# fabsig/GPBoost

Hardware: AMD Instinct MI355X
Metric: neg-log-lik evals/sec, n=1000000 Vecchia(m=30) fp64 (higher is better)
Workload: dtype f64

## Files before the change

### gpboost_amd/csrc/dev_common.h

```cpp
#pragma once
#include <hip/hip_runtime.h>
#include <stdint.h>
#include <type_traits>
#include <utility>

namespace gpb {

template <int B, int E, class F>
__device__ __forceinline__ void static_for(F&& f) {
  if constexpr (B < E) {
    f(std::integral_constant<int, B>{});
    static_for<B + 1, E>(f);
  }
}
template <int B, int E, class F>
__device__ __forceinline__ void static_for_down(F&& f) {
  if constexpr (B < E) {
    f(std::integral_constant<int, E - 1>{});
    static_for_down<B, E - 1>(f);
  }
}

template <int LANE>
__device__ __forceinline__ double row_bcast(double x) {
  static_assert(LANE >= 0 && LANE < 16, "row_newbcast lane");
  double r;
  asm volatile("s_nop 1\n\tv_mov_b64_dpp %0, %1 row_newbcast:%2 row_mask:0xf bank_mask:0xf"
               : "=v"(r)
               : "v"(x), "n"(LANE));
  return r;
}
template <int LANE>
__device__ __forceinline__ void row_fnma(double& acc, double b, double own) {
  static_assert(LANE >= 0 && LANE < 16, "row_newbcast lane");
#ifdef GPB_DPP_PAD_EVERY_FMAC
  asm volatile("s_nop 1\n\tv_fmac_f64_dpp %0, -%1, %2 row_newbcast:%3 row_mask:0xf bank_mask:0xf"
               : "+v"(acc)
               : "v"(b), "v"(own), "n"(LANE));
#else
  asm volatile("v_fmac_f64_dpp %0, -%1, %2 row_newbcast:%3 row_mask:0xf bank_mask:0xf"
               : "+v"(acc)
               : "v"(b), "v"(own), "n"(LANE));
#endif
}
__device__ __forceinline__ void dpp_fence(double& a) { asm volatile("s_nop 1" : "+v"(a)); }
__device__ __forceinline__ void dpp_fence(double& a, double& b) { asm volatile("s_nop 1" : "+v"(a), "+v"(b)); }
__device__ __forceinline__ void dpp_fence(double& a, double& b, double& c) { asm volatile("s_nop 1" : "+v"(a), "+v"(b), "+v"(c)); }
__device__ __forceinline__ void dpp_fence(double& a, double& b, double& c, double& d) { asm volatile("s_nop 1" : "+v"(a), "+v"(b), "+v"(c), "+v"(d)); }
template <int CTRL>
__device__ __forceinline__ double dpp_move_f64(double v) {
  const long long b = __builtin_bit_cast(long long, v);
  int lo = (int)(b & 0xffffffffll), hi = (int)(b >> 32);
  lo = __builtin_amdgcn_update_dpp(0, lo, CTRL, 0xF, 0xF, true);
  hi = __builtin_amdgcn_update_dpp(0, hi, CTRL, 0xF, 0xF, true);
  return __builtin_bit_cast(double, ((long long)hi << 32) | (long long)(unsigned int)lo);
}
__device__ __forceinline__ double row_sum16(double v) {
  v += dpp_move_f64<0xB1>(v);
  v += dpp_move_f64<0x4E>(v);
  v += dpp_move_f64<0x141>(v);
  v += dpp_move_f64<0x140>(v);
  return v;
}
__host__ __device__ constexpr unsigned long long row_lanes_le(int j) {
  return j < 0 ? 0ull : (j >= 15 ? ~0ull : ((1ull << (j + 1)) - 1ull) * 0x0001000100010001ull);
}
__host__ __device__ constexpr unsigned long long row_lane_eq(int j) { return (1ull << j) * 0x0001000100010001ull; }
template <unsigned long long MASK>
__device__ __forceinline__ int sel_lanes(int a, int b, int tok) {
  int r;
  asm("s_mov_b32 vcc_lo, %3\n\ts_mov_b32 vcc_hi, %4\n\tv_cndmask_b32_e32 %0, %1, %2, vcc ; %5"
      : "=v"(r) : "v"(b), "v"(a), "n"((int)(unsigned)(MASK & 0xffffffffull)), "n"((int)(unsigned)(MASK >> 32)), "s"(tok) : "vcc");
  return r;
}
template <unsigned long long MASK, int A, int B>
__device__ __forceinline__ int sel_lanes_const(int tok) {
  static_assert(A >= 0 && A <= 64 && B >= 0 && B <= 64, "inline constants only");
  int r;
  asm("s_mov_b32 vcc_lo, %3\n\ts_mov_b32 vcc_hi, %4\n\tv_cndmask_b32_e64 %0, %1, %2, vcc ; %5"
      : "=v"(r) : "n"(B), "n"(A), "n"((int)(unsigned)(MASK & 0xffffffffull)), "n"((int)(unsigned)(MASK >> 32)), "s"(tok) : "vcc");
  return r;
}
template <unsigned long long MASK>
__device__ __forceinline__ void set_lanes(double& dst, double v) {
  asm volatile("s_mov_b32 exec_lo, %2\n\ts_mov_b32 exec_hi, %3\n\tv_mov_b64 %0, %1\n\ts_mov_b64 exec, -1"
               : "+v"(dst) : "v"(v), "n"((int)(unsigned)(MASK & 0xffffffffull)), "n"((int)(unsigned)(MASK >> 32)));
}
template <int LANE>
__device__ __forceinline__ double row_bcast_builtin(double x) {
  const long long v = __builtin_bit_cast(long long, x);
  int lo = (int)(v & 0xffffffffll), hi = (int)(v >> 32);
  lo = __builtin_amdgcn_update_dpp(0, lo, 0x150 + LANE, 0xf, 0xf, false);
  hi = __builtin_amdgcn_update_dpp(0, hi, 0x150 + LANE, 0xf, 0xf, false);
  const long long r = ((long long)hi << 32) | (unsigned long long)(unsigned int)lo;
  return __builtin_bit_cast(double, r);
}
#ifdef GPB_DPP_VIA_BUILTIN
#define GPB_ROW_BCAST(L, x) ::gpb::row_bcast_builtin<L>(x)
#define GPB_ROW_FNMA(L, acc, b, own) (acc) = __builtin_fma(-::gpb::row_bcast_builtin<L>(b), (own), (acc))
#else
#define GPB_ROW_BCAST(L, x) ::gpb::row_bcast<L>(x)
#define GPB_ROW_FNMA(L, acc, b, own) ::gpb::row_fnma<L>((acc), (b), (own))
#endif


__device__ __forceinline__ double fast_rcp(double x) {
  const double y0 = __builtin_amdgcn_rcp(x);
  const double e = __builtin_fma(-x, y0, 1.0);
  return __builtin_fma(y0, e, y0);
}

#ifndef GPB_EXP_TAB_SIZE
#define GPB_EXP_TAB_SIZE 256
#endif
static_assert(GPB_EXP_TAB_SIZE == 256, "exp_of_scaled is written for a 256-entry table");

enum CovType : int { kMatern05 = 0, kMatern15 = 1, kMatern25 = 2 };

constexpr double kLn2OverT = 0.0027076061740622863;
constexpr double kCoordScale = 184.6649652337873;

struct KernEval { double ev, rp; };
__device__ __forceinline__ KernEval exp_of_scaled(double d2q, const double* __restrict__ tabv) {
  const double h = __builtin_amdgcn_rsq(d2q);
  const double g = d2q * h;
  const double e = __builtin_fma(-h, g, 3.0);
  const double rp = g * e;
  const double kf = __builtin_rint(-rp);
  const double rr = -rp - kf;
  const int k = (int)kf;
  double p = __builtin_fma(rr, 2.239395190875157e-12, 3.3083026805413713e-09);
  p = __builtin_fma(p, rr, 3.6655655969101062e-06);
  p = __builtin_fma(p, rr, kLn2OverT);
  p = __builtin_fma(p, rr, 1.0);
  KernEval o;
  o.ev = __builtin_ldexp(tabv[k & (GPB_EXP_TAB_SIZE - 1)] * p, k >> 8);
  o.rp = rp;
  return o;
}
template <int COV>
__device__ __forceinline__ double matern_cov_s(double d2s, const double* __restrict__ tabv) {
  const KernEval k = exp_of_scaled(d2s, tabv);
  if constexpr (COV == kMatern05) return k.ev;
  else if constexpr (COV == kMatern15) return k.ev * __builtin_fma(k.rp, kLn2OverT, 1.0);
  else { const double r = k.rp * kLn2OverT; return k.ev * __builtin_fma(r, __builtin_fma(r, 1.0 / 3.0, 1.0), 1.0); }
}
template <int COV>
__device__ __forceinline__ double matern_cov_dlog_s(double d2s, const double* __restrict__ tabv, double& dk) {
  const KernEval k = exp_of_scaled(d2s, tabv);
  const double r = k.rp * kLn2OverT;
  if constexpr (COV == kMatern05) { dk = -r * k.ev; return k.ev; }
  else if constexpr (COV == kMatern15) { dk = -(r * r) * k.ev; return k.ev * (1.0 + r); }
  else { dk = -(1.0 / 3.0) * (r * r) * (1.0 + r) * k.ev; return k.ev * __builtin_fma(r, __builtin_fma(r, 1.0 / 3.0, 1.0), 1.0); }
}
template <int COV>
__device__ __forceinline__ double matern_dlog_range_s(double d2s, const double* __restrict__ tabv) {
  const KernEval k = exp_of_scaled(d2s, tabv);
  const double r = k.rp * kLn2OverT;
  if constexpr (COV == kMatern05) return -r * k.ev;
  else if constexpr (COV == kMatern15) return -(r * r) * k.ev;
  else return -(1.0 / 3.0) * (r * r) * __builtin_fma(1.0, r, 1.0) * k.ev;
}

}
```

### gpboost_amd/csrc/vecchia_kernels.hip

```cpp
#include <algorithm>
#include "dev_common.h"
#include "vecchia_kernels.h"

namespace gpb {

namespace {

constexpr double kDummyCoord = 1e30;

__host__ __device__ constexpr int lane_of_row(int r) { return ((r / 16) & 1) ? 15 - (r % 16) : (r % 16); }

template <int MT>
struct Layout {
  static_assert(MT >= 1 && MT <= 62, "1 <= MT <= 62");
  static_assert(MT % 16 != 15, "row MT and row MT+1 must share a register slot");
  static constexpr int R = MT + 2;
  static constexpr int NS = (R + 15) / 16;
  static constexpr int PS = MT / 16, PL = lane_of_row(MT);
  static constexpr int YS = (MT + 1) / 16, YL = lane_of_row(MT + 1);
  static constexpr int NCOL = MT + 1;
  static constexpr int PTS_BYTES32 = (NS * 16) * 32 + 16;
  static constexpr int PTS_STRIDE24 = NS * 16 + 2;
  __host__ __device__ static constexpr int cmax(int s) { return (16 * s + 15 < MT) ? 16 * s + 15 : MT; }
};

template <bool D3> struct RecT;
template <> struct RecT<true> { double x, y, z, w; __device__ __forceinline__ double zz() const { return z; } };
template <> struct RecT<false> { double x, y, w; __device__ __forceinline__ double zz() const { return 0.0; } };

template <bool D3>
__device__ __forceinline__ double sq_dist_s(double px, double py, double pz, double qx, double qy, double qz) {
  const double dx = px - qx, dy = py - qy;
  double d2 = __builtin_fma(dx, dx, 1e-300);
  d2 = __builtin_fma(dy, dy, d2);
  if constexpr (D3) {
    const double dz = pz - qz;
    d2 = __builtin_fma(dz, dz, d2);
  }
  return d2;
}

template <int MT>
__host__ __device__ constexpr int num_lower_steps() {
  using L = Layout<MT>;
  int n = 8 * L::NS * (L::NS - 1) + 15 * (L::NS / 2);
  if (L::NS & 1) { const int s = L::NS - 1; const int chi = (16 * s + 14 < MT - 1) ? 16 * s + 14 : MT - 1; n += chi - 16 * s + 1; }
  return n;
}
template <int MT, class FR, class FP, class FS>
__device__ __forceinline__ void for_each_lower_step(FR&& rect, FP&& pair, FS&& solo) {
  using L = Layout<MT>;
  constexpr int RECT_TOTAL = 8 * L::NS * (L::NS - 1);
  static_for<1, L::NS>([&](auto s_) {
    constexpr int s = decltype(s_)::value;
    static_for<0, 16 * s>([&](auto c_) { rect(s_, c_, std::integral_constant<int, 8 * s * (s - 1) + decltype(c_)::value>{}); });
  });
  static_for<0, L::NS>([&](auto s_) {
    constexpr int s = decltype(s_)::value;
    if constexpr ((s & 1) == 1) {
      static_for<0, 15>([&](auto j_) {
        constexpr int j = decltype(j_)::value;
        constexpr int cA = 16 * s + j, cB = 16 * (s - 1) + 14 - j;
        using E = std::integral_constant<int, RECT_TOTAL + 15 * (s / 2) + j>;
        if constexpr (cA <= MT - 1) pair(s_, std::integral_constant<int, cA>{}, std::integral_constant<int, s - 1>{},
                                         std::integral_constant<int, cB>{}, std::integral_constant<int, 14 - j>{}, E{});
        else solo(std::integral_constant<int, s - 1>{}, std::integral_constant<int, cB>{}, E{});
      });
    } else if constexpr (s == L::NS - 1) {
      constexpr int chi = (16 * s + 14 < MT - 1) ? 16 * s + 14 : MT - 1;
      static_for<16 * s, chi + 1>([&](auto c_) { solo(s_, c_, std::integral_constant<int, RECT_TOTAL + 15 * (L::NS / 2) + decltype(c_)::value - 16 * s>{}); });
    }
  });
}

}

constexpr unsigned long long kGranuleEmpty = ~0ull;
template <int NP>
__device__ __forceinline__ void vecchia_finish(const VecchiaKernelArgs& args, int G, double (*s_fin)[4]);

template <int MT, int MODE>
constexpr bool kRuntimeWeightedInstance() { return MODE == MODE_GRAD && MT > 30 && MT <= 40; }

template <int MT, int COV, bool D3, int MODE, bool WT>
__global__ __launch_bounds__(256, (MT > 30 && MT <= 40 && MODE != MODE_NLL) ? 2 : 1) void vecchia_point_kernel(VecchiaKernelArgs args) {
  using L = Layout<MT>;
  constexpr int NS = L::NS;
  constexpr bool kNeedSolve = (MODE != MODE_NLL);
#ifdef GPB_NLL_RIGHT_LOOKING
  constexpr bool kLeftLooking = false;
#else
  constexpr bool kLeftLooking = MT > 30 && (!kNeedSolve || NS == 3);
#endif
  constexpr bool kLeftSolve = kLeftLooking && kNeedSolve;
  constexpr int NP = (MODE == MODE_GRAD) ? GPB_NUM_PARTIALS : 3;

  using Rec = RecT<D3>;
  constexpr bool kStoreDK = (MODE == MODE_GRAD) && (MT <= 30);
  constexpr int NSTEP = num_lower_steps<MT>();
  constexpr bool kLastDkInReg = kStoreDK && D3;
  constexpr int NSTORE = kStoreDK ? (kLastDkInReg ? NSTEP - 1 : NSTEP) : 1;
  constexpr int PBYTES = D3 ? L::PTS_BYTES32 : L::PTS_STRIDE24 * (int)sizeof(Rec);
  __shared__ double s_tab[GPB_EXP_TAB_SIZE];
  __shared__ __attribute__((aligned(16))) char s_pts_raw[16 * PBYTES];
  __shared__ double s_red[GPB_NUM_PARTIALS][16];
  __shared__ double s_f0[kLeftSolve ? 16 : 1][kLeftSolve ? 256 : 1];
  constexpr bool kDgInLds = WT && (MODE == MODE_NLL) && kLeftLooking;
  __shared__ double s_dg[kDgInLds ? 16 : 1][kDgInLds ? NS * 16 : 1];
  __shared__ double s_dk[NSTORE][kStoreDK ? 256 : 1];
  static_assert(PBYTES % 16 == 0 && PBYTES >= 16 * (NS * 16), "record block: 16-byte aligned, room for the (A, b) pairs");
  __shared__ double2 s_ab[(MODE == MODE_GRAD && !kStoreDK) ? 16 : 1][(MODE == MODE_GRAD && !kStoreDK) ? NS * 16 : 1];
  double dk_last = 0.0;

  __shared__ double s_tot[GPB_NUM_PARTIALS];
  __shared__ double s_fin[GPB_NUM_PARTIALS][4];

  const int G = (int)gridDim.x - 1;
  if ((int)blockIdx.x == G) { vecchia_finish<NP>(args, G, s_fin); return; }
  const int tid0 = threadIdx.x;
  static_assert(GPB_EXP_TAB_SIZE == 256, "one table entry per thread");
  s_tab[tid0] = args.exp_tab[tid0] * args.var;
  if (tid0 < NP) s_tot[tid0] = 0.0;
  __shared__ double s_pm[16];
  __shared__ int s_pe[16];
  if (tid0 < 16) { s_pm[tid0] = 0.5; s_pe[tid0] = 1; }

  const int m = args.m;
  auto fetch_idx = [&](int grp_, int tid_, int (&out)[NS]) {
    const int g_ = tid_ >> 4, l_ = tid_ & 15;
    const long long ir = (long long)args.i_begin + (long long)grp_ * 16 + g_;
    const int ii = ir < (long long)args.i_end ? (int)ir : args.i_end - 1;
#pragma unroll
    for (int s = 0; s < NS; ++s) {
      const int r = 16 * s + ((s & 1) ? 15 - l_ : l_);
      int idx = -1;
      if (r < m) idx = args.nn[(size_t)ii * m + r];
      else if (r == MT) idx = ii;
      out[s] = idx;
    }
  };
  int nidx[NS];
  fetch_idx(blockIdx.x, tid0, nidx);
  for (int grp = blockIdx.x; grp < args.ngroups; grp += G) {
  int tid = tid0;
  asm volatile("; per-trip thread index" : "+v"(tid));
  const int g = tid >> 4;
  const int l = tid & 15;
  const long long i_raw = (long long)args.i_begin + (long long)grp * 16 + g;
  const bool active = i_raw < (long long)args.i_end;
  const int i = active ? (int)i_raw : args.i_end - 1;
  int cidx[NS];
#pragma unroll
  for (int s = 0; s < NS; ++s) cidx[s] = nidx[s];
  if (grp + G < args.ngroups) fetch_idx(grp + G, tid, nidx);
  const double sc = args.a * kCoordScale;

  const double4 ctr = args.pts[i];
  Rec own[NS];
  constexpr bool kRuntimeW = WT && kRuntimeWeightedInstance<MT, MODE>();
  const bool weighted = kRuntimeW ? (args.nug != nullptr) : WT;
  constexpr int kOwnDg = (kDgInLds || !WT) ? 1 : NS;
  double own_dg[kOwnDg];
#pragma unroll
  for (int s = 0; s < kOwnDg; ++s) own_dg[s] = 0.0;
  auto own_dg_of = [&](int s) -> double { if constexpr (kOwnDg == NS) return own_dg[s]; else { (void)s; return own_dg[0]; } };
#pragma unroll
  for (int s = 0; s < NS; ++s) {
    const int r = 16 * s + ((s & 1) ? 15 - l : l);
    const int idx = cidx[s];
    if (WT && weighted) {
      const double dgv = args.var + (idx >= 0 ? args.nug[idx] : 1.0);
      if constexpr (kDgInLds) s_dg[g][r] = dgv; else own_dg[s] = dgv;
    }
    Rec p;
    if (idx >= 0) {
      const double4 q = args.pts[idx];
      p.x = (q.x - ctr.x) * sc; p.y = (q.y - ctr.y) * sc; p.w = q.w;
      if constexpr (D3) p.z = (q.z - ctr.z) * sc;
    } else {
      p.x = kDummyCoord * (double)(r + 1); p.y = 0.0; p.w = 0.0;
      if constexpr (D3) p.z = 0.0;
    }
    own[s] = p;
    reinterpret_cast<Rec*>(s_pts_raw + g * PBYTES)[r] = p;
  }
  __syncthreads();
  const double* tabv = s_tab;
  const Rec* gp = reinterpret_cast<const Rec*>(s_pts_raw + g * PBYTES);
  int row_off[NS];
#pragma unroll
  for (int s = 0; s < NS; ++s) row_off[s] = (16 * s + ((s & 1) ? 15 - l : l)) * (int)sizeof(Rec);

  double M[NS][L::NCOL];
  auto eval_entry = [&](const Rec& o, const Rec& q, auto e_) -> double {
    const double d2 = sq_dist_s<D3>(o.x, o.y, o.zz(), q.x, q.y, q.zz());
    if constexpr (kStoreDK) {
      double dk;
      const double v = matern_cov_dlog_s<COV>(d2, tabv, dk);
      if constexpr (kLastDkInReg && decltype(e_)::value == NSTEP - 1) dk_last = dk;
      else s_dk[decltype(e_)::value][tid] = dk;
      return v;
    } else {
      return matern_cov_s<COV>(d2, tabv);
    }
  };
  if constexpr (kLeftLooking) {
    auto eval_plain = [&](const Rec& o, const Rec& q) -> double {
      return matern_cov_s<COV>(sq_dist_s<D3>(o.x, o.y, o.zz(), q.x, q.y, q.zz()), tabv);
    };
    static_for<0, MT + 1>([&](auto c_) {
      constexpr int c = decltype(c_)::value;
      constexpr int sc_ = c / 16, lc = lane_of_row(c);
      if constexpr (c < MT) {
        static_for<sc_ + 1, NS>([&](auto s_) { constexpr int s = decltype(s_)::value; M[s][c] = eval_plain(own[s], gp[c]); });
        if constexpr ((c % 16) != 15 && (sc_ & 1) == 0) {
          constexpr int j = 14 - (c - 16 * sc_);
          constexpr int sA = sc_ + 1, cA = 16 * sA + j;
          if constexpr (sA < NS && cA <= MT - 1) {
            constexpr unsigned long long MA = row_lanes_le(14 - j);
            const int ro = sel_lanes<MA>(row_off[sA], row_off[sc_], grp);
            const int co = sel_lanes_const<MA, cA, c>(grp) * (int)sizeof(Rec);
            const double v = eval_plain(*reinterpret_cast<const Rec*>(reinterpret_cast<const char*>(gp) + ro),
                                        *reinterpret_cast<const Rec*>(reinterpret_cast<const char*>(gp) + co));
            M[sA][cA] = v;
            M[sc_][c] = v;
          } else {
            M[sc_][c] = eval_plain(own[sc_], gp[c]);
          }
        }
      }
      {
        double dg;
        if constexpr (kDgInLds) dg = weighted ? s_dg[g][c] : ((c == MT) ? args.diag_i : args.diag_nn);
        else dg = weighted ? own_dg_of(sc_) : ((c == MT) ? args.diag_i : args.diag_nn);
        if constexpr (c == 16 * sc_ + 15 || c == MT) M[sc_][c] = dg;
        else set_lanes<row_lane_eq(lc)>(M[sc_][c], dg);
        set_lanes<row_lane_eq(L::YL)>(M[L::YS][c], gp[c].w);
      }
      static_for<0, c>([&](auto k_) {
        constexpr int k = decltype(k_)::value;
        static_for<sc_, NS>([&](auto s_) {
          constexpr int s = decltype(s_)::value;
          GPB_ROW_FNMA(lc, M[s][c], M[sc_][k], M[s][k]);
        });
      });
      if constexpr (c < MT) {
        const double piv = GPB_ROW_BCAST(lc, M[sc_][c]);
        const double y0 = __builtin_amdgcn_rsq(piv);
        const double e = __builtin_fma(-0.5 * piv * y0, y0, 0.5);
        const double rs = __builtin_fma(y0, e, y0);
        static_for<sc_, NS>([&](auto s_) { constexpr int s = decltype(s_)::value; M[s][c] *= rs; });
        if constexpr (kLeftSolve) set_lanes<row_lane_eq(lc)>(M[sc_][c], rs);
        static_assert(NS <= 4, "dpp_fence overloads cover four slots");
        if constexpr (NS - sc_ == 1) dpp_fence(M[sc_][c]);
        else if constexpr (NS - sc_ == 2) dpp_fence(M[sc_][c], M[sc_ + 1][c]);
        else if constexpr (NS - sc_ == 3) dpp_fence(M[sc_][c], M[sc_ + 1][c], M[sc_ + 2][c]);
        else dpp_fence(M[sc_][c], M[sc_ + 1][c], M[sc_ + 2][c], M[sc_ + 3][c]);
        if constexpr (kLeftSolve && c == 15) static_for<0, 16>([&](auto q_) { s_f0[decltype(q_)::value][tid] = M[0][decltype(q_)::value]; });
      }
    });
  } else {
  for_each_lower_step<MT>(
      [&](auto s_, auto c_, auto e_) {
        constexpr int s = decltype(s_)::value, c = decltype(c_)::value;
        M[s][c] = eval_entry(own[s], gp[c], e_);
      },
      [&](auto sA_, auto cA_, auto sB_, auto cB_, auto J_, auto e_) {
        constexpr int sA = decltype(sA_)::value, cA = decltype(cA_)::value, sB = decltype(sB_)::value,
                      cB = decltype(cB_)::value, J = decltype(J_)::value;
        constexpr unsigned long long MA = row_lanes_le(J);
        const int ro = sel_lanes<MA>(row_off[sA], row_off[sB], grp);
        const int co = sel_lanes_const<MA, cA, cB>(grp) * (int)sizeof(Rec);
        const Rec o = *reinterpret_cast<const Rec*>(reinterpret_cast<const char*>(gp) + ro);
        const Rec q = *reinterpret_cast<const Rec*>(reinterpret_cast<const char*>(gp) + co);
        const double v = eval_entry(o, q, e_);
        M[sA][cA] = v;
        M[sB][cB] = v;
      },
      [&](auto s_, auto c_, auto e_) {
        constexpr int s = decltype(s_)::value, c = decltype(c_)::value;
        M[s][c] = eval_entry(own[s], gp[c], e_);
      });
  static_for<0, NS>([&](auto s_) {
    constexpr int s = decltype(s_)::value;
    static_for<16 * s, L::cmax(s) + 1>([&](auto c_) {
      constexpr int c = decltype(c_)::value;
      double dg;
      if constexpr (kDgInLds) dg = weighted ? s_dg[g][c] : ((c == MT) ? args.diag_i : args.diag_nn);
      else dg = weighted ? own_dg_of(s) : ((c == MT) ? args.diag_i : args.diag_nn);
      if constexpr (c == 16 * s + 15 || c == MT) M[s][c] = dg;
      else set_lanes<row_lane_eq(lane_of_row(c))>(M[s][c], dg);
    });
  });
  if (l == L::YL) {
    static_for<0, MT + 1>([&](auto c_) { M[L::YS][decltype(c_)::value] = gp[decltype(c_)::value].w; });
  }

  static_for<0, MT>([&](auto k_) {
    constexpr int k = decltype(k_)::value;
    constexpr int sk = k / 16, lk = lane_of_row(k);
    if constexpr (k == 0) static_for<0, NS>([&](auto s_) { dpp_fence(M[decltype(s_)::value][0]); });
    const double piv = GPB_ROW_BCAST(lk, M[sk][k]);
    const double inv = fast_rcp(piv);
    double T[NS];
    static_for<sk, NS>([&](auto s_) { T[decltype(s_)::value] = M[decltype(s_)::value][k] * inv; });
    static_for<k + 1, MT + 1>([&](auto c_) {
      constexpr int c = decltype(c_)::value;
      constexpr int sc_ = c / 16, lc = lane_of_row(c);
      static_for<sc_, NS>([&](auto s_) {
        constexpr int s = decltype(s_)::value;
        GPB_ROW_FNMA(lc, M[s][c], M[sc_][k], T[s]);
      });
    });
    if constexpr (kNeedSolve) static_for<sk, NS>([&](auto s_) { M[decltype(s_)::value][k] = T[decltype(s_)::value]; });
  });
  }

  const double Dv = GPB_ROW_BCAST(L::PL, M[L::PS][MT]);
  const double uv = GPB_ROW_BCAST(L::YL, M[L::YS][MT]);
  const double Dinv = 1.0 / Dv;

  double red[GPB_NUM_PARTIALS];
#pragma unroll
  for (int t = 0; t < GPB_NUM_PARTIALS; ++t) red[t] = 0.0;
  red[GPB_P_LOGDET] = Dv;
  red[GPB_P_QUAD] = uv * uv * Dinv;
  red[GPB_P_BAD] = (Dv > 0.0) ? 0.0 : 1.0;

  if constexpr (kNeedSolve) {
    constexpr bool kLaneX = MT > 30;
    double X[kLaneX ? 1 : MT];
    double xa[NS], xb[NS];
    if constexpr (kLeftSolve) {
      static_assert(NS == 3 && L::PS == 2 && L::YS == 2, "kLeftSolve: three slots, the point's and the response row in the last one");
#pragma unroll
      for (int s = 0; s < NS; ++s) { xa[s] = 0.0; xb[s] = 0.0; }
      static_for_down<0, MT>([&](auto k_) {
        constexpr int k = decltype(k_)::value;
        constexpr int sk = k / 16, lk = lane_of_row(k);
        constexpr unsigned long long kKeep = (sk & 1) ? row_lanes_le(14 - (k % 16)) : ~row_lanes_le(k % 16);
        double own_col;
        if constexpr (sk == 0) own_col = s_f0[k][tid]; else own_col = M[sk][k];
        double ta = own_col * xa[sk], tb = own_col * xb[sk];
        set_lanes<~kKeep>(ta, 0.0);
        set_lanes<~kKeep>(tb, 0.0);
        static_for<sk + 1, NS>([&](auto s_) {
          constexpr int s = decltype(s_)::value;
          ta = __builtin_fma(M[s][k], xa[s], ta);
          tb = __builtin_fma(M[s][k], xb[s], tb);
        });
        ta = row_sum16(ta); tb = row_sum16(tb);
        const double rk = GPB_ROW_BCAST(lk, own_col);
        const double la = GPB_ROW_BCAST(L::PL, M[L::PS][k]);
        const double lb = GPB_ROW_BCAST(L::YL, M[L::YS][k]);
        set_lanes<row_lane_eq(lk)>(xa[sk], (la - ta) * rk);
        set_lanes<row_lane_eq(lk)>(xb[sk], (lb - tb) * rk);
      });
    } else if constexpr (kLaneX) {
#pragma unroll
      for (int s = 0; s < NS; ++s) { xa[s] = 0.0; xb[s] = 0.0; }
      static_for_down<0, MT>([&](auto k_) {
        constexpr int k = decltype(k_)::value;
        constexpr int sk = k / 16, lk = lane_of_row(k);
        constexpr unsigned long long kKeep = (sk & 1) ? row_lanes_le(14 - (k % 16)) : ~row_lanes_le(k % 16);
        double ta = M[sk][k] * xa[sk], tb = M[sk][k] * xb[sk];
        set_lanes<~kKeep>(ta, 0.0);
        set_lanes<~kKeep>(tb, 0.0);
        static_for<sk + 1, NS>([&](auto s_) {
          constexpr int s = decltype(s_)::value;
          ta = __builtin_fma(M[s][k], xa[s], ta);
          tb = __builtin_fma(M[s][k], xb[s], tb);
        });
        ta = row_sum16(ta); tb = row_sum16(tb);
        const double la = GPB_ROW_BCAST(L::PL, M[L::PS][k]);
        const double lb = GPB_ROW_BCAST(L::YL, M[L::YS][k]);
        set_lanes<row_lane_eq(lk)>(xa[sk], la - ta);
        set_lanes<row_lane_eq(lk)>(xb[sk], lb - tb);
      });
    } else {
    static_for<0, MT>([&](auto k_) { X[decltype(k_)::value] = M[L::PS][decltype(k_)::value]; });
    static_for<0, MT>([&](auto k_) { static_for<0, NS>([&](auto s_) { if constexpr (decltype(k_)::value <= L::cmax(decltype(s_)::value)) dpp_fence(M[decltype(s_)::value][decltype(k_)::value]); }); });
    static_for_down<0, MT>([&](auto j_) {
      constexpr int j = decltype(j_)::value;
      constexpr int sj = j / 16, lj = lane_of_row(j);
      static_for_down<0, j>([&](auto k_) {
        constexpr int k = decltype(k_)::value;
        GPB_ROW_FNMA(lj, X[k], M[sj][k], X[j]);
      });
    });
    }
    if constexpr (MODE == MODE_FACTOR) {
      if constexpr (kLaneX) {
        if (active) {
          double* Arow = args.A + (size_t)i * m;
#pragma unroll
          for (int s = 0; s < NS; ++s) { const int r = 16 * s + ((s & 1) ? 15 - l : l); if (r < m) Arow[r] = xa[s]; }
        }
      } else {
      if (active && l == L::PL) {
        double* Arow = args.A + (size_t)i * m;
        static_for<0, MT>([&](auto k_) {
          constexpr int k = decltype(k_)::value;
          if (k < m) Arow[k] = X[k];
        });
      }
      }
      if (active && l == 0) { args.D[i] = Dv; args.u[i] = uv; }
    }
    if constexpr (MODE == MODE_GRAD) {
      asm volatile("" ::: "memory");
      double2* gab = kStoreDK ? reinterpret_cast<double2*>(s_pts_raw + g * PBYTES) : &s_ab[g][0];
      if constexpr (kLaneX) {
#pragma unroll
        for (int s = 0; s < NS; ++s) {
          const int r = 16 * s + ((s & 1) ? 15 - l : l);
          gab[r] = r < MT ? make_double2(xa[s], xb[s]) : (r == MT ? make_double2(-1.0, 0.0) : make_double2(0.0, 0.0));
        }
      } else {
      if (l == L::PL) { static_for<0, MT>([&](auto k_) { gab[decltype(k_)::value].x = X[decltype(k_)::value]; }); gab[MT].x = -1.0; gab[MT + 1].x = 0.0; }
      if (l == L::YL) { static_for<0, MT>([&](auto k_) { gab[decltype(k_)::value].y = X[decltype(k_)::value]; }); gab[MT].y = 0.0; gab[MT + 1].y = 0.0; }
      if (l == 0) { for (int r = MT + 2; r < NS * 16; ++r) gab[r] = make_double2(0.0, 0.0); }
      }
      __syncthreads();
      double2 abr[NS];
      int ab_off[NS];
      double sAA = 0.0, sbA = 0.0;
      static_for<0, NS>([&](auto s_) {
        constexpr int s = decltype(s_)::value;
        const int r = 16 * s + ((s & 1) ? 15 - l : l);
        abr[s] = gab[r]; ab_off[s] = r * (int)sizeof(double2);
        const double nr = weighted ? own_dg_of(s) - args.var : 1.0;
        if (r < MT) { sAA = __builtin_fma(nr * abr[s].x, abr[s].x, sAA); sbA = __builtin_fma(nr * abr[s].y, abr[s].x, sbA); }
      });
      double accD = 0.0, accU = 0.0;
      auto accumulate = [&](double dk, const double2& r_, const double2& c_) {
        accD = __builtin_fma(dk * r_.x, c_.x, accD);
        accU = __builtin_fma(dk, __builtin_fma(r_.y, c_.x, c_.y * r_.x), accU);
      };
      auto dk_of = [&](auto e_, const Rec& o, const Rec& q) -> double {
        if constexpr (kStoreDK) {
          if constexpr (kLastDkInReg && decltype(e_)::value == NSTEP - 1) return dk_last;
          else return s_dk[decltype(e_)::value][tid];
        } else {
          return matern_dlog_range_s<COV>(sq_dist_s<D3>(o.x, o.y, o.zz(), q.x, q.y, q.zz()), tabv);
        }
      };
      for_each_lower_step<MT>(
          [&](auto s_, auto c_, auto e_) {
            constexpr int s = decltype(s_)::value, c = decltype(c_)::value;
            if constexpr (kStoreDK) accumulate(dk_of(e_, own[s], gp[c]), abr[s], gab[c]);
            else accumulate(dk_of(e_, *reinterpret_cast<const Rec*>(reinterpret_cast<const char*>(gp) + row_off[s]), gp[c]), abr[s], gab[c]);
          },
          [&](auto sA_, auto cA_, auto sB_, auto cB_, auto J_, auto e_) {
            constexpr int sA = decltype(sA_)::value, cA = decltype(cA_)::value, sB = decltype(sB_)::value,
                          cB = decltype(cB_)::value, J = decltype(J_)::value;
            constexpr unsigned long long MA = row_lanes_le(J);
            const int ci = sel_lanes_const<MA, cA, cB>(grp);
            double dk;
            if constexpr (kStoreDK) dk = dk_of(e_, own[0], own[0]);
            else {
              const int ro = sel_lanes<MA>(row_off[sA], row_off[sB], grp);
              dk = dk_of(e_, *reinterpret_cast<const Rec*>(reinterpret_cast<const char*>(gp) + ro),
                         *reinterpret_cast<const Rec*>(reinterpret_cast<const char*>(gp) + ci * (int)sizeof(Rec)));
            }
            const int ao = sel_lanes<MA>(ab_off[sA], ab_off[sB], grp);
            accumulate(dk, *reinterpret_cast<const double2*>(reinterpret_cast<const char*>(gab) + ao), gab[ci]);
          },
          [&](auto s_, auto c_, auto e_) {
            constexpr int s = decltype(s_)::value, c = decltype(c_)::value;
            static_assert((s & 1) == 0, "solo steps only occur in even slots");
            double dk;
            if constexpr (kStoreDK) dk = dk_of(e_, own[s], gp[c]);
            else dk = dk_of(e_, *reinterpret_cast<const Rec*>(reinterpret_cast<const char*>(gp) + row_off[s]), gp[c]);
            set_lanes<row_lanes_le(c - 16 * s)>(dk, 0.0);
            accumulate(dk, abr[s], gab[c]);
          });
#pragma unroll
      for (int off = 8; off >= 1; off >>= 1) {
        accD += __shfl_xor(accD, off, 16);
        accU += __shfl_xor(accU, off, 16);
        sAA += __shfl_xor(sAA, off, 16);
        sbA += __shfl_xor(sbA, off, 16);
      }
      const double up = uv * Dinv;
      double nug_i = args.nugget;
      if (WT && weighted) nug_i = args.nug[i];
      const double dD_var = Dv - nug_i - sAA;
      const double uk_var = -sbA;
      const double dD_rng = 2.0 * accD;
      const double uk_rng = accU;
      red[GPB_P_G1_VAR] = uk_var * up - 0.5 * up * up * dD_var;
      red[GPB_P_G2_VAR] = 0.5 * Dinv * dD_var;
      red[GPB_P_G1_RNG] = uk_rng * up - 0.5 * up * up * dD_rng;
      red[GPB_P_G2_RNG] = 0.5 * Dinv * dD_rng;
    }
  }

  if (l == 0) {
#pragma unroll
    for (int t = 0; t < NP; ++t) s_red[t][g] = active ? red[t] : (t == GPB_P_LOGDET ? 1.0 : 0.0);
  }
  __syncthreads();
  if (tid < 16) {
    const double dv = s_red[GPB_P_LOGDET][tid];
    const double p = s_pm[tid] * __builtin_amdgcn_frexp_mant(dv);
    s_pm[tid] = (dv > 0.0) ? __builtin_amdgcn_frexp_mant(p) : __builtin_nan("");
    s_pe[tid] += __builtin_amdgcn_frexp_exp(dv) + __builtin_amdgcn_frexp_exp(p);
  } else if (tid >= 64 && tid < 64 + NP && tid - 64 != GPB_P_LOGDET) {
    const int t = tid - 64;
    double acc = 0.0;
#pragma unroll
    for (int q = 0; q < 16; ++q) acc += s_red[t][q];
    s_tot[t] += acc;
  }
  }
  const int tid = tid0;
  __syncthreads();
  if (tid < 16) s_red[GPB_P_LOGDET][tid] = log(s_pm[tid]) + (double)s_pe[tid] * 0.693147180559945309417232121458;
  __syncthreads();
  if (tid == 0) {
    double acc = 0.0;
#pragma unroll
    for (int q = 0; q < 16; ++q) acc += s_red[GPB_P_LOGDET][q];
    s_tot[GPB_P_LOGDET] = acc;
  }
  __syncthreads();

  if (tid < NP)
    __hip_atomic_store(reinterpret_cast<unsigned long long*>(args.partials + (size_t)tid * G + blockIdx.x),
                       (unsigned long long)__double_as_longlong(s_tot[tid]), __ATOMIC_RELAXED, __HIP_MEMORY_SCOPE_AGENT);
}

template <int NP>
__device__ __forceinline__ void vecchia_finish(const VecchiaKernelArgs& args, int G, double (*s_fin)[4]) {
  const int tid = threadIdx.x;
#pragma unroll
  for (int t = 0; t < NP; ++t) {
    double acc = 0.0, comp = 0.0;
    unsigned long long* base = reinterpret_cast<unsigned long long*>(args.partials + (size_t)t * G);
    constexpr int kBatch = 8;
    for (int b0 = tid; b0 < G; b0 += 256 * kBatch) {
      unsigned long long raw[kBatch];
#pragma unroll
      for (int q = 0; q < kBatch; ++q) {
        const int b = b0 + 256 * q;
        raw[q] = b < G ? __hip_atomic_load(base + b, __ATOMIC_RELAXED, __HIP_MEMORY_SCOPE_AGENT) : 0ull;
      }
#pragma unroll
      for (int q = 0; q < kBatch; ++q) {
        const int b = b0 + 256 * q;
        if (b >= G) break;
        while (raw[q] == kGranuleEmpty) {
          __builtin_amdgcn_s_sleep(8);
          raw[q] = __hip_atomic_load(base + b, __ATOMIC_RELAXED, __HIP_MEMORY_SCOPE_AGENT);
        }
        __hip_atomic_store(base + b, kGranuleEmpty, __ATOMIC_RELAXED, __HIP_MEMORY_SCOPE_AGENT);
        const double v = __longlong_as_double((long long)raw[q]) - comp;
        const double tmp = acc + v;
        comp = (tmp - acc) - v;
        acc = tmp;
      }
    }
#pragma unroll
    for (int off = 32; off >= 1; off >>= 1) acc += __shfl_xor(acc, off, 64);
    if ((tid & 63) == 0) s_fin[t][tid >> 6] = acc;
  }
  __syncthreads();
  if (tid < NP) {
    const double v = (s_fin[tid][0] + s_fin[tid][1]) + (s_fin[tid][2] + s_fin[tid][3]);
    args.out[tid] = v;
    if (args.out_user) args.out_user[tid == GPB_P_LOGDET ? 1 : (tid == GPB_P_QUAD ? 0 : tid)] = v;
    if (args.out_host) __hip_atomic_store(reinterpret_cast<unsigned long long*>(args.out_host + tid), (unsigned long long)__double_as_longlong(v),
                                          __ATOMIC_RELAXED, __HIP_MEMORY_SCOPE_SYSTEM);
  }
}


#ifdef GPB_INSTANTIATE_MT
#ifndef GPB_INSTANTIATE_MODE
#error "define GPB_INSTANTIATE_MODE (0 nll, 1 factor, 2 grad) together with GPB_INSTANTIATE_MT"
#endif
template <int MT, int COV, bool D3, bool WT>
static int persistent_grid(const VecchiaKernelArgs& args) {
  auto kern = vecchia_point_kernel<MT, COV, D3, GPB_INSTANTIATE_MODE, WT>;
  static int cached_dev = -1, per_dev = 0;
  int dev = 0;
  if (hipGetDevice(&dev) != hipSuccess) return args.ngroups;
  if (dev != cached_dev) {
    int occ = 0, cus = 0;
    if (hipOccupancyMaxActiveBlocksPerMultiprocessor(&occ, kern, 256, 0) != hipSuccess || occ < 1) occ = 1;
    if (hipDeviceGetAttribute(&cus, hipDeviceAttributeMultiprocessorCount, dev) != hipSuccess || cus < 1) cus = 256;
    per_dev = occ * cus; cached_dev = dev;
    (void)hipGetLastError();
  }
  const int auto_rounds = (int)std::max(1LL, std::min(8LL, ((long long)args.ngroups + 2LL * per_dev) / (4LL * per_dev)));
  const long long slots = (long long)per_dev * auto_rounds;
  if (args.ngroups <= slots) return args.ngroups;
  const int trips = (int)((args.ngroups + slots - 1) / slots);
  return (args.ngroups + trips - 1) / trips;
}
template <int MT, bool D3>
static hipError_t launch_cov(int cov, const VecchiaKernelArgs& args, int nblocks, hipStream_t st) {
  (void)nblocks;
  switch (cov) {
#define GPB_LAUNCH_COV(C) \
  if (args.nug || kRuntimeWeightedInstance<MT, GPB_INSTANTIATE_MODE>()) hipLaunchKernelGGL((vecchia_point_kernel<MT, C, D3, GPB_INSTANTIATE_MODE, true>), dim3(persistent_grid<MT, C, D3, true>(args) + 1), dim3(256), 0, st, args); \
  else hipLaunchKernelGGL((vecchia_point_kernel<MT, C, D3, GPB_INSTANTIATE_MODE, false>), dim3(persistent_grid<MT, C, D3, false>(args) + 1), dim3(256), 0, st, args); \
  break
    case kMatern05: GPB_LAUNCH_COV(kMatern05);
    case kMatern15: GPB_LAUNCH_COV(kMatern15);
    case kMatern25: GPB_LAUNCH_COV(kMatern25);
#undef GPB_LAUNCH_COV
    default: return hipErrorInvalidValue;
  }
  return hipGetLastError();
}
#define GPB_CAT4_(a, b, c, d) a##b##c##d
#define GPB_CAT4(a, b, c, d) GPB_CAT4_(a, b, c, d)
hipError_t GPB_CAT4(launch_vecchia_mt, GPB_INSTANTIATE_MT, _mode, GPB_INSTANTIATE_MODE)(bool d3, int cov, const VecchiaKernelArgs& args,
                                                                                      int nblocks, hipStream_t st) {
  return d3 ? launch_cov<GPB_INSTANTIATE_MT, true>(cov, args, nblocks, st)
            : launch_cov<GPB_INSTANTIATE_MT, false>(cov, args, nblocks, st);
}
#else
#define GPB_CASE(MTV)                                                                                   \
  hipError_t launch_vecchia_mt##MTV##_mode0(bool, int, const VecchiaKernelArgs&, int, hipStream_t);       \
  hipError_t launch_vecchia_mt##MTV##_mode1(bool, int, const VecchiaKernelArgs&, int, hipStream_t);       \
  hipError_t launch_vecchia_mt##MTV##_mode2(bool, int, const VecchiaKernelArgs&, int, hipStream_t);
GPB_MT_CASES
#undef GPB_CASE

int vecchia_padded_m(int m) {
  const int sizes[] = {GPB_MT_LIST};
  for (int s : sizes) if (m <= s) return s;
  return -1;
}

hipError_t launch_vecchia_point_kernel(int mode, int cov, bool d3, const VecchiaKernelArgs& args, hipStream_t st) {
  const int npts = args.i_end - args.i_begin;
  if (npts <= 0) return hipErrorInvalidValue;
  const int nblocks = (npts + 15) / 16;
  if (args.ngroups != nblocks || !args.out) return hipErrorInvalidValue;
  const int mt = vecchia_padded_m(args.m);
  switch (mt) {
#define GPB_CASE(MTV)                                                                       \
  case MTV:                                                                                   \
    if (mode == MODE_NLL) return launch_vecchia_mt##MTV##_mode0(d3, cov, args, nblocks, st);  \
    if (mode == MODE_FACTOR) return launch_vecchia_mt##MTV##_mode1(d3, cov, args, nblocks, st); \
    if (mode == MODE_GRAD) return launch_vecchia_mt##MTV##_mode2(d3, cov, args, nblocks, st);  \
    return hipErrorInvalidValue;
    GPB_MT_CASES
#undef GPB_CASE
    default: return hipErrorInvalidValue;
  }
}

#endif

}
```

Baseline: 1071.

## Replace per-trip workgroup barriers with wave-level ordering and batched partial replay

For neighbor counts between 20 and 40, the kernel now replaces the workgroup-wide barriers around the per-group LDS point and A/b staging with a wave-scope fence and wave barrier. This relies on each 16-lane group's LDS data being produced and consumed within the same wavefront. Per-trip partial results are written into an LDS history ring whose depth is sized from the LDS budget. The log-determinant and sum reductions are replayed only every kDepth trips, and once more at the end, instead of after every trip. This removes most block-wide synchronisation from the grid-stride loop, at the cost of extra LDS and a correctness dependency on wave-local data ownership.

```diff
diff --git a/gpboost_amd/csrc/dev_common.h b/gpboost_amd/csrc/dev_common.h
--- a/gpboost_amd/csrc/dev_common.h
+++ b/gpboost_amd/csrc/dev_common.h
@@ -61,6 +61,11 @@
   v += dpp_move_f64<0x141>(v);
   v += dpp_move_f64<0x140>(v);
   return v;
+}
+__device__ __forceinline__ void wave_lds_order() {
+  __builtin_amdgcn_fence(__ATOMIC_ACQ_REL, "wavefront");
+  __builtin_amdgcn_wave_barrier();
+  __builtin_amdgcn_fence(__ATOMIC_ACQ_REL, "wavefront");
 }
 __host__ __device__ constexpr unsigned long long row_lanes_le(int j) {
   return j < 0 ? 0ull : (j >= 15 ? ~0ull : ((1ull << (j + 1)) - 1ull) * 0x0001000100010001ull);
diff --git a/gpboost_amd/csrc/vecchia_kernels.hip b/gpboost_amd/csrc/vecchia_kernels.hip
--- a/gpboost_amd/csrc/vecchia_kernels.hip
+++ b/gpboost_amd/csrc/vecchia_kernels.hip
@@ -103,7 +103,6 @@
   constexpr int PBYTES = D3 ? L::PTS_BYTES32 : L::PTS_STRIDE24 * (int)sizeof(Rec);
   __shared__ double s_tab[GPB_EXP_TAB_SIZE];
   __shared__ __attribute__((aligned(16))) char s_pts_raw[16 * PBYTES];
-  __shared__ double s_red[GPB_NUM_PARTIALS][16];
   __shared__ double s_f0[kLeftSolve ? 16 : 1][kLeftSolve ? 256 : 1];
   constexpr bool kDgInLds = WT && (MODE == MODE_NLL) && kLeftLooking;
   __shared__ double s_dg[kDgInLds ? 16 : 1][kDgInLds ? NS * 16 : 1];
@@ -114,6 +113,16 @@
 
   __shared__ double s_tot[GPB_NUM_PARTIALS];
   __shared__ double s_fin[GPB_NUM_PARTIALS][4];
+  constexpr bool kFreeTrips = MT >= 20 && MT <= 40;
+  constexpr int kLdsOther = GPB_EXP_TAB_SIZE * 8 + 16 * PBYTES + (kLeftSolve ? 16 * 256 * 8 : 8) + (kDgInLds ? 16 * NS * 16 * 8 : 8) +
+                            NSTORE * (kStoreDK ? 256 * 8 : 8) + ((MODE == MODE_GRAD && !kStoreDK) ? 16 * NS * 16 * 16 : 16) +
+                            GPB_NUM_PARTIALS * 8 + GPB_NUM_PARTIALS * 4 * 8 + 16 * 8 + 16 * 4;
+  constexpr int kLdsPerCu = 160 * 1024;
+  constexpr int kLdsWgs = (kLdsPerCu / kLdsOther < 8) ? kLdsPerCu / kLdsOther : 8;
+  constexpr int kLdsRoom = kLdsPerCu / kLdsWgs - kLdsOther - 256;
+  constexpr int kDepth = !kFreeTrips ? 1 : (kLdsRoom >= 8 * NP * 128) ? 8 : ((kLdsRoom >= NP * 128) ? kLdsRoom / (NP * 128) : 1);
+  static_assert(kDepth == 1 || kLdsOther + kDepth * NP * 128 <= kLdsPerCu / kLdsWgs, "the history must not cost a workgroup per CU");
+  __shared__ double s_hist[kDepth][kFreeTrips ? NP : GPB_NUM_PARTIALS][16];
 
   const int G = (int)gridDim.x - 1;
   if ((int)blockIdx.x == G) { vecchia_finish<NP>(args, G, s_fin); return; }
@@ -139,8 +148,34 @@
       out[s] = idx;
     }
   };
+  auto replay = [&](int tid_, int nslots) {
+    if (tid_ < 16) {
+      double pm = s_pm[tid_];
+      int pe = s_pe[tid_];
+      for (int sl = 0; sl < nslots; ++sl) {
+        const double dv = s_hist[sl][GPB_P_LOGDET][tid_];
+        const double p = pm * __builtin_amdgcn_frexp_mant(dv);
+        pm = (dv > 0.0) ? __builtin_amdgcn_frexp_mant(p) : __builtin_nan("");
+        pe += __builtin_amdgcn_frexp_exp(dv) + __builtin_amdgcn_frexp_exp(p);
+      }
+      s_pm[tid_] = pm;
+      s_pe[tid_] = pe;
+    } else if (tid_ >= 64 && tid_ < 64 + NP && tid_ - 64 != GPB_P_LOGDET) {
+      const int t = tid_ - 64;
+      double tot = s_tot[t];
+      for (int sl = 0; sl < nslots; ++sl) {
+        double acc = 0.0;
+#pragma unroll
+        for (int q = 0; q < 16; ++q) acc += s_hist[sl][t][q];
+        tot += acc;
+      }
+      s_tot[t] = tot;
+    }
+  };
   int nidx[NS];
   fetch_idx(blockIdx.x, tid0, nidx);
+  if constexpr (kFreeTrips) __syncthreads();
+  int slot = 0;
   for (int grp = blockIdx.x; grp < args.ngroups; grp += G) {
   int tid = tid0;
   asm volatile("; per-trip thread index" : "+v"(tid));
@@ -184,7 +219,7 @@
     own[s] = p;
     reinterpret_cast<Rec*>(s_pts_raw + g * PBYTES)[r] = p;
   }
-  __syncthreads();
+  if constexpr (kFreeTrips) wave_lds_order(); else __syncthreads();
   const double* tabv = s_tab;
   const Rec* gp = reinterpret_cast<const Rec*>(s_pts_raw + g * PBYTES);
   int row_off[NS];
@@ -421,7 +456,7 @@
       if (l == L::YL) { static_for<0, MT>([&](auto k_) { gab[decltype(k_)::value].y = X[decltype(k_)::value]; }); gab[MT].y = 0.0; gab[MT + 1].y = 0.0; }
       if (l == 0) { for (int r = MT + 2; r < NS * 16; ++r) gab[r] = make_double2(0.0, 0.0); }
       }
-      __syncthreads();
+      if constexpr (kFreeTrips) wave_lds_order(); else __syncthreads();
       double2 abr[NS];
       int ab_off[NS];
       double sAA = 0.0, sbA = 0.0;
@@ -498,11 +533,21 @@
 
   if (l == 0) {
 #pragma unroll
-    for (int t = 0; t < NP; ++t) s_red[t][g] = active ? red[t] : (t == GPB_P_LOGDET ? 1.0 : 0.0);
-  }
+    for (int t = 0; t < NP; ++t) s_hist[slot][t][g] = active ? red[t] : (t == GPB_P_LOGDET ? 1.0 : 0.0);
+  }
+  if constexpr (kFreeTrips) {
+  ++slot;
+  wave_lds_order();
+  if (slot == kDepth && grp + G < args.ngroups) {
+    __syncthreads();
+    replay(tid, kDepth);
+    __syncthreads();
+    slot = 0;
+  }
+  } else {
   __syncthreads();
   if (tid < 16) {
-    const double dv = s_red[GPB_P_LOGDET][tid];
+    const double dv = s_hist[0][GPB_P_LOGDET][tid];
     const double p = s_pm[tid] * __builtin_amdgcn_frexp_mant(dv);
     s_pm[tid] = (dv > 0.0) ? __builtin_amdgcn_frexp_mant(p) : __builtin_nan("");
     s_pe[tid] += __builtin_amdgcn_frexp_exp(dv) + __builtin_amdgcn_frexp_exp(p);
@@ -510,18 +555,20 @@
     const int t = tid - 64;
     double acc = 0.0;
 #pragma unroll
-    for (int q = 0; q < 16; ++q) acc += s_red[t][q];
+    for (int q = 0; q < 16; ++q) acc += s_hist[0][t][q];
     s_tot[t] += acc;
+  }
   }
   }
   const int tid = tid0;
   __syncthreads();
-  if (tid < 16) s_red[GPB_P_LOGDET][tid] = log(s_pm[tid]) + (double)s_pe[tid] * 0.693147180559945309417232121458;
+  if constexpr (kFreeTrips) replay(tid, slot);
+  if (tid < 16) s_hist[0][GPB_P_LOGDET][tid] = log(s_pm[tid]) + (double)s_pe[tid] * 0.693147180559945309417232121458;
   __syncthreads();
   if (tid == 0) {
     double acc = 0.0;
 #pragma unroll
-    for (int q = 0; q < 16; ++q) acc += s_red[GPB_P_LOGDET][q];
+    for (int q = 0; q < 16; ++q) acc += s_hist[0][GPB_P_LOGDET][q];
     s_tot[GPB_P_LOGDET] = acc;
   }
   __syncthreads();
```

Result: no change. 1079, median of 6 (+0.7%).
